# Improbable-AI/walk-these-ways

Hardware: NVIDIA H100
Metric: env_steps_per_s (higher is better)
Workload: dtype tf32

## Files before the change

include/go1_b200.h:

```cpp
#ifndef GO1_B200_H
#define GO1_B200_H
#include <stdint.h>
#ifdef __cplusplus
extern "C" {
#endif

#define GO1_NUM_DOF 12
#define GO1_NUM_COMMANDS 15
#define GO1_MAX_OBS 128
#define GO1_MAX_PRIV_OBS 48
#define GO1_EVENT_STRIDE 6
#define GO1_RESET_RAND_STRIDE 48
#define GO1_MAX_LAG_TIMESTEPS 32

enum Go1RewardTerm {
    GO1_REW_TRACKING_LIN_VEL = 0, GO1_REW_TRACKING_ANG_VEL, GO1_REW_LIN_VEL_Z, GO1_REW_ANG_VEL_XY,
    GO1_REW_ORIENTATION, GO1_REW_TORQUES, GO1_REW_DOF_ACC, GO1_REW_ACTION_RATE, GO1_REW_COLLISION,
    GO1_REW_DOF_POS_LIMITS, GO1_REW_JUMP, GO1_REW_TRACKING_CONTACTS_SHAPED_FORCE,
    GO1_REW_TRACKING_CONTACTS_SHAPED_VEL, GO1_REW_DOF_POS, GO1_REW_DOF_VEL, GO1_REW_ACTION_SMOOTHNESS_1,
    GO1_REW_ACTION_SMOOTHNESS_2, GO1_REW_FEET_SLIP, GO1_REW_FEET_CONTACT_VEL, GO1_REW_FEET_CONTACT_FORCES,
    GO1_REW_FEET_CLEARANCE_CMD_LINEAR, GO1_REW_FEET_IMPACT_VEL, GO1_REW_ORIENTATION_CONTROL,
    GO1_REW_RAIBERT_HEURISTIC, GO1_REW_TERMINATION, GO1_NUM_REWARD_TERMS
};

// ... 195 lines not shown
} Go1TailProblem;
int go1_mlp_tail_forward_grouped(const Go1TailProblem* probs, int nprob, int M, int K1, int N2, int N3, void* stream);

int go1_gemm_timing(int on, double* total_ms, double* total_flop, long long* launches);
void go1_kernel_launch_add(long long n);
int go1_transpose(const float* src, int lds, float* dst, int ldd, int rows, int cols, void* stream);
int go1_elu_backward(const float* y, int ldy, const float* dy, int lddy, float* dz, int lddz, int M, int N, void* stream);
int go1_act_backward(const float* y, int ldy, const float* dy, int lddy, float* dz, int lddz, int M, int N, int kind, void* stream);
int go1_mlp_extra_forward(float* y, int ldy, const float* extra, int ldex, const float* w_extra, int ldw, int M, int o, int E, int act,
                          void* stream);
int go1_mlp_extra_backward(const float* dz, int lddz, int dz_transposed, const float* extra, int ldex, const float* w_extra, int ldw,
                           float* g_w_extra, int ldgw, float* dextra, int ldde, int M, int o, int E, int accumulate, void* stream);
int go1_skinny_forward(const float* x, int ldx, const float* W, int ldw, const float* b, float* out, int ldo, int M, int o, int K, void* stream);
int go1_skinny_dgrad(const float* dz, int lddz, const float* W, int ldw, const float* y_prev, int ldy, float* dprev, int lddp,
                     int M, int o, int n, void* stream);
int go1_skinny_dgrad_ex(const float* dz, int lddz, const float* W, int ldw, const float* y_prev, int ldy, float* dprev, int lddp,
                        float* colsum, int M, int o, int n, void* stream);
int go1_skinny_dgrad_act(const float* dz, int lddz, const float* W, int ldw, const float* y_prev, int ldy, float* dprev, int lddp,
                         float* colsum, int M, int o, int n, int kind, void* stream);
int go1_skinny_wgrad_ex(const float* dz, int lddz, const float* x, int ldx, float* gW, int ldg, float* gb, int M, int o, int K, int accumulate, void* stream);
int go1_skinny_wgrad(const float* dz, int lddz, const float* x, int ldx, float* gW, int ldg, int M, int o, int K, int accumulate, void* stream);
typedef struct Go1CopySeg { const float* src; int32_t lds; float* dst; int32_t ldd; int32_t rows, cols; } Go1CopySeg;
int go1_copy_segments(const Go1CopySeg* segs, int n, void* stream);
int go1_colsum(const float* x, int ldx, float* out, int M, int N, int accumulate, void* stream);

int go1_ppo_sample_actions(const float* mean, int ldm, const float* std, const float* eps, uint64_t seed,
                           uint64_t counter, uint64_t* counter_dev, float* actions, float* logp, int n, int num_actions,
                           void* stream);

int go1_ppo_loss(const float* mean, int ldm, const float* std, const float* value, const float* actions,
                 const float* old_logp, const float* old_mean, const float* old_std, const float* advantages,
                 const float* returns, const float* old_values, float* dmean, int lddm, float* dvalue,
                 float* dstd, float* scalars, int n, int num_actions, float clip_param,
                 float value_loss_coef, float entropy_coef, int use_clipped_value_loss, float inv_count,
                 void* stream);

int go1_ppo_mse(const float* pred, int ldp, const float* target, int ldt, float* dpred, int lddp, float* scalars,
                int n, int num_train, int dim, void* stream);

int go1_ppo_grad_sqnorm(const float* grad, int64_t count, double* grad_sq, void* stream);
int go1_ppo_adam_step(float* param, const float* grad, float* exp_avg, float* exp_avg_sq, int64_t count,
                      const double* grad_sq, float max_grad_norm, float lr, const float* lr_dev, float beta1, float beta2,
                      float eps, int step, void* stream);
int go1_ppo_adaptive_lr(const float* scalars, float* lr_dev, float desired_kl, float lr_min, float lr_max, void* stream);

int go1_store_transition(const float* const* in_f32, const uint8_t* dones, const uint8_t* time_outs, float* const* out_f32, uint8_t* s_dones,
// ... 18 lines not shown
```

walk-these-ways_b200/csrc/gemm_tf32.cu:

```cuda
#include <cuda_runtime.h>
#include <cuda.h>
#include <stdint.h>
#include <stdio.h>
#include <mutex>
#include <unordered_map>
#include <stdlib.h>
#include "../../include/go1_b200.h"
#include "wgmma_tf32.cuh"
#include "activation.cuh"

extern int go1_set_error(const char* m);
void go1_count_launch(int n);

namespace {

constexpr int BM = 128, BK = 32;
constexpr int NCONS = 8, EPI_G = 2;

__device__ __forceinline__ uint32_t smem_u32(const void* p) { return (uint32_t)__cvta_generic_to_shared(p); }

__device__ __forceinline__ void mbar_init(uint64_t* bar, uint32_t count) {
    asm volatile("mbarrier.init.shared::cta.b64 [%0], %1;" ::"r"(smem_u32(bar)), "r"(count));
}
__device__ __forceinline__ void mbar_expect_tx(uint64_t* bar, uint32_t bytes) {
// ... 65 lines not shown


struct GemmArgs {
    float* C; const float* bias;
    int M, N, K, ldc, act, kind, accumulate, kb_per_split;
    const float* ex; const float* wex; const float* aux;
    int ldex, ldwex, nex, ldaux;
    int lead;
    int amn, bmn;
    int ct;
    float* colsum;
    const float* bx; const float* bwx; float* gwx; float* dx;
    int ldbx, ldbwx, ldgwx, lddx, nbx;
    int tma_store, tma_aux;
    float* Cg[4]; int nprob, tiles_per_prob;
};
constexpr int GEMM_MAXP = 4;
struct GemmMaps { CUtensorMap a[GEMM_MAXP], b[GEMM_MAXP], half; };

struct EpiStage {
    uint8_t* out;
    const CUtensorMap* mapC;
    const uint8_t* aux;
};
__device__ __forceinline__ void tma_store_2d(const CUtensorMap* map, const void* src, int c0, int c1) {
    asm volatile("cp.async.bulk.tensor.2d.global.shared::cta.bulk_group [%0, {%2, %3}], [%1];"
                 ::"l"(map), "r"(smem_u32(src)), "r"(c0), "r"(c1) : "memory");
}

template <typename D>
__device__ __forceinline__ void epilogue_dact(const D dact, const GemmArgs& g, float (&v)[32], const int row, const int col0, const int ncols, const int lane,
                                              const float4 (&ypre)[8], const bool have_pre, const EpiStage& es) {
    const float* arow = g.aux + (size_t)row * g.ldaux + col0;
    if (es.aux) {
        const uint8_t* srow = es.aux + lane * 128;
#pragma unroll
        for (int j = 0; j < 8; j++) {
            const float4 y = *reinterpret_cast<const float4*>(srow + ((j ^ (lane & 7)) << 4));
            v[4 * j] *= dact(y.x); v[4 * j + 1] *= dact(y.y); v[4 * j + 2] *= dact(y.z); v[4 * j + 3] *= dact(y.w);
        }
    } else if (have_pre) {
#pragma unroll
        for (int j = 0; j < 8; j++) {
            const float4 y = ypre[j];
            v[4 * j] *= dact(y.x); v[4 * j + 1] *= dact(y.y); v[4 * j + 2] *= dact(y.z); v[4 * j + 3] *= dact(y.w);
        }
// ... 82 lines not shown
    }
    if (g.bias) {
        const float bl = cj < g.N ? __ldg(g.bias + cj) : 0.f;
#pragma unroll
        for (int j = 0; j < 32; j++) v[j] += __shfl_sync(0xffffffffu, bl, j);
    }
    const int kind = ANYKIND ? g.kind : (int)GO1_ACT_ELU;
    if (row_ok) {
    if (g.act == 1) {
        const int nlead = g.lead <= 0 ? 32 : max(0, min(32, g.lead - col0));
        GO1_ACT_SWITCH(kind, KD,
            _Pragma("unroll")
            for (int j = 0; j < 32; j++) if (j < nlead) v[j] = act_fast<KD>(v[j]);)
    } else if (g.act == 2) {
        if (ANYKIND) epilogue_dact(act_deriv_coefficients(kind), g, v, row, col0, ncols, lane, ypre, have_pre, es);
        else epilogue_dact([](float y) { return act_deriv<GO1_ACT_ELU>(y); }, g, v, row, col0, ncols, lane, ypre, have_pre, es);
    }
    }
    if (g.colsum) {
        float sred[32];
#pragma unroll
        for (int j = 0; j < 32; j++) sred[j] = (row_ok && j < ncols) ? v[j] : 0.f;
        const float s = transpose_reduce32(sred, lane);
        if (lane < ncols) atomicAdd(g.colsum + col0 + lane, s);
    }
    if (g.nbx > 0) {
        const int cjx = col0 + lane;
#pragma unroll
        for (int t = 0; t < 4; t++) {
            if (t < g.nbx) {
                if (g.gwx) {
                const float e = row_ok ? __ldg(g.bx + (size_t)row * g.ldbx + t) : 0.f;
                float sred[32];
#pragma unroll
                for (int j = 0; j < 32; j++) sred[j] = (row_ok && j < ncols) ? v[j] * e : 0.f;
                const float s = transpose_reduce32(sred, lane);
                if (lane < ncols) atomicAdd(g.gwx + (size_t)cjx * g.ldgwx + t, s);
                }
                if (g.dx) {
                    const float wl = lane < ncols ? __ldg(g.bwx + (size_t)cjx * g.ldbwx + t) : 0.f;
                    float acc = 0.f;
#pragma unroll
                    for (int j = 0; j < 32; j++) acc = fmaf(v[j], __shfl_sync(0xffffffffu, wl, j), acc);
                    if (row_ok) atomicAdd(g.dx + (size_t)row * g.lddx + t, acc);
                }
            }
        }
// ... 17 lines not shown
            else tma_store_2d(es.mapC, es.out, col0, row);
            asm volatile("cp.async.bulk.commit_group;" ::: "memory");
        }
        return;
    }
    if (!row_ok) return;
    if (vec) {
#pragma unroll
        for (int j = 0; j < 8; j++) reinterpret_cast<float4*>(crow)[j] = make_float4(v[4 * j], v[4 * j + 1], v[4 * j + 2], v[4 * j + 3]);
    } else {
#pragma unroll
        for (int j = 0; j < 32; j++) if (j < ncols) crow[j] = v[j];
    }
}

__device__ __forceinline__ bool epilogue_prefetch(const GemmArgs& g, const int row, const int col0, const bool split, float4 (&ypre)[8]) {
    if (g.act != 2 || split || col0 + 32 > g.N || (g.ldaux & 3) != 0 || ((((uintptr_t)g.aux) & 15) != 0) || (col0 & 3) != 0) return false;
    const float4* arow = reinterpret_cast<const float4*>(g.aux + (size_t)(row < g.M ? row : 0) * g.ldaux + col0);
#pragma unroll
    for (int j = 0; j < 8; j++) ypre[j] = __ldg(arow + j);
    return true;
}

constexpr int X_BYTES = 65536;
template <int BN, bool ANYKIND, int CL>
__global__ void __launch_bounds__(32 * NCONS + 128, 1) gemm_tf32_wgmma(const __grid_constant__ GemmMaps gm,
                                                                      const __grid_constant__ CUtensorMap mapC, const __grid_constant__ CUtensorMap mapY, const GemmArgs g,
                                                                      const int tiles_m, const int tiles_n, const int total_tiles, const int stages) {
    static_assert(CL == 1 || (CL == 2 && BN == BM), "CTA pairs share 128-row operand boxes");
    constexpr int G = EPI_G;
    constexpr int A_BYTES = BM * BK * 4, STAGE_BYTES = (BM + BN) * BK * 4;
    constexpr int MAX_STAGES = 8;
    extern __shared__ __align__(1024) uint8_t smem_raw[];
    uint8_t* base = (uint8_t*)(((uintptr_t)smem_raw + 1023) & ~(uintptr_t)1023);
    uint8_t* ring = base;
    uint8_t* xreg = base + (size_t)stages * STAGE_BYTES;
    uint8_t* stage_aux = xreg + X_BYTES;
    uint64_t* full = (uint64_t*)(stage_aux + (g.tma_aux ? NCONS * 4096 : 0));
    uint64_t* empty = full + MAX_STAGES;
    uint64_t* aux_bar = empty + MAX_STAGES;

    const int warp = threadIdx.x >> 5, lane = threadIdx.x & 31;
    const int num_kb_total = (g.K + BK - 1) / BK;

    if (threadIdx.x == 0) {
        for (int p = 0; p < g.nprob; p++) {
            asm volatile("prefetch.tensormap [%0];" ::"l"(&gm.a[p]) : "memory");
            asm volatile("prefetch.tensormap [%0];" ::"l"(&gm.b[p]) : "memory");
        }
        if (g.tma_store) asm volatile("prefetch.tensormap [%0];" ::"l"(&mapC) : "memory");
        if (g.tma_aux) asm volatile("prefetch.tensormap [%0];" ::"l"(&mapY) : "memory");
        if (CL > 1) asm volatile("prefetch.tensormap [%0];" ::"l"(&gm.half) : "memory");
        for (int s = 0; s < stages; s++) { mbar_init(&full[s], 1); mbar_init(&empty[s], CL * NCONS); }
        for (int w = 0; w < NCONS; w++) mbar_init(&aux_bar[w], 1);
        asm volatile("fence.mbarrier_init.release.cluster;" ::: "memory");
    }
    if (CL > 1) cluster_sync();
    else __syncthreads();

    const int npt = total_tiles / CL;
    auto first = [] { return (int)blockIdx.x / CL; };
    auto step = [] { return (int)gridDim.x / CL; };
    auto rank = [] { return CL > 1 ? cluster_ctarank() : 0u; };
    auto pair_n = [&] { return (tiles_n & 1) == 0; };
    auto cta_tile = [&](int pt) -> int {
        if (CL == 1) return pt;
        if (pair_n()) return 2 * pt + (int)rank();
        const int tn = pt % tiles_n, r = pt / tiles_n, hm = tiles_m / 2;
        return ((r / hm) * tiles_m + 2 * (r % hm) + (int)rank()) * tiles_n + tn;
    };
    auto tile_coords = [&](int t, int& m0, int& n0, int& kb0, int& nkb) {
        if (CL == 1 && g.nprob > 1) t %= g.tiles_per_prob;
        const int tn = t % tiles_n; t /= tiles_n;
        const int tm = t % tiles_m; const int z = t / tiles_m;
        m0 = tm * BM; n0 = tn * BN; kb0 = z * g.kb_per_split; nkb = min(g.kb_per_split, num_kb_total - kb0);
    };

    if (warp == NCONS) {
        if (elect_one()) {
// ... 55 lines not shown
    };
    auto release = [&](int s) {
        if (lane == 0) {
            mbar_arrive(&empty[s]);
            if (CL > 1) mbar_arrive_cluster(&empty[s], rank() ^ 1);
        }
    };
    auto request_aux = [&]() {
        if (next_chunk() && lane == 0) {
            int m0, n0, kb0, nkb; tile_coords(cta_tile(pt), m0, n0, kb0, nkb);
            mbar_expect_tx(my_bar, 4096);
            tma_load_2d(&mapY, my_bar, my_aux, n0 + 32 * pc, m0 + 32 * q);
        }
    };
    if (st_aux) request_aux();
    uint32_t aux_phase = 0;
    int s = 0, ph = 0;
    float acc[BN / 2];
    for (int tp = first(); tp < npt; tp += step()) {
        const int t = cta_tile(tp);
        int m0, n0, kb0, nkb; tile_coords(t, m0, n0, kb0, nkb);
        if (st_out && lane == 0) asm volatile("cp.async.bulk.wait_group.read 0;" ::: "memory");
        cons_sync();
        int prev = -1;
        for (int i = 0; i < nkb; i++) {
            mbar_wait(&full[s], ph);
            const uint8_t* a = ring + (size_t)s * STAGE_BYTES;
            const uint8_t* b = a + A_BYTES;
            if (tr) {
                if (g.amn) { uint8_t* ta = xreg + (i & 1) * A_BYTES; transpose_tile<BM>((const float*)a, ta, ctid); a = ta; }
                if (g.bmn) { uint8_t* tb = xreg + 2 * A_BYTES + (i & 1) * A_BYTES; transpose_tile<BN>((const float*)b, tb, ctid); b = tb; }
                if (prev >= 0) {
                    wg::wait<0>();
                    release(prev);
                }
                fence_async_smem();
                cons_sync();
            }
            wg::fence();
            wg::mma_kblock<BN>(acc, a + (size_t)wgi * 64 * 128, b, i > 0);
            wg::commit();
            if (!tr && prev >= 0) {
                wg::wait<1>();
                release(prev);
            }
            prev = s;
// ... 1 lines not shown
        }
        wg::wait<0>();
        release(prev);
        if (tr) cons_sync();

        const int row = m0 + 32 * q + lane;
        float* const Cbase = CL == 1 && g.nprob > 1 ? g.Cg[t / g.tiles_per_prob] : g.C;
        float4 ypre[8];
        const bool have_pre = CL == 1 && !st_aux && (grp < BN / 32) && epilogue_prefetch(g, row, n0 + 32 * grp, split, ypre);
        store_fragment<BN / 8>(acc, xwg, 0, w, lane, [](float2 v, int, int) { return v; });
        wg_sync(wgi);
#pragma unroll 1
        for (int c = grp; c < BN / 32; c += G) {
            if (n0 + 32 * c >= g.N) break;
            uint8_t* blk = xwg + (size_t)c * (64 * 128) + (w & 1) * 4096;
            uint32_t r[32];
            const uint8_t* srow = blk + lane * 128;
#pragma unroll
            for (int j = 0; j < 8; j++) {
                const uint4 x = *reinterpret_cast<const uint4*>(srow + ((j ^ (lane & 7)) << 4));
                r[4 * j] = x.x; r[4 * j + 1] = x.y; r[4 * j + 2] = x.z; r[4 * j + 3] = x.w;
            }
            EpiStage es;
            es.out = st_out ? blk : nullptr; es.mapC = &mapC; es.aux = st_aux ? my_aux : nullptr;
            if (st_aux) { mbar_wait(my_bar, aux_phase); aux_phase ^= 1; }
            epilogue_chunk<ANYKIND>(g, Cbase, r, row, n0 + 32 * c, split, lane, ypre, have_pre && c == grp, es);
            if (st_aux) { __syncwarp(); request_aux(); }
        }
    }
    if (st_out && lane == 0) asm volatile("cp.async.bulk.wait_group 0;" ::: "memory");
    if (CL > 1) cluster_sync();
}

typedef CUresult (*EncodeTiledFn)(CUtensorMap*, CUtensorMapDataType, cuuint32_t, void*, const cuuint64_t*, const cuuint64_t*, const cuuint32_t*,
                                  const cuuint32_t*, CUtensorMapInterleave, CUtensorMapSwizzle, CUtensorMapL2promotion, CUtensorMapFloatOOBfill);
EncodeTiledFn g_encode = nullptr;
std::once_flag g_once;

int sm_count() {
    static int sms = 0;
    if (!sms) { int dev = 0; cudaGetDevice(&dev); cudaDeviceGetAttribute(&sms, cudaDevAttrMultiProcessorCount, dev); if (sms <= 0) sms = 132; }
    return sms;
}

int make_map_uncached(CUtensorMap* map, const float* ptr, int rows, int cols, int ld, int box_rows, int box_cols, CUtensorMapSwizzle swz);
struct MapKey { const float* ptr; int rows, cols, ld, box_rows, box_cols, swz; bool operator==(const MapKey& o) const { return ptr == o.ptr && rows == o.rows && cols == o.cols && ld == o.ld && box_rows == o.box_rows && box_cols == o.box_cols && swz == o.swz; } };
struct MapKeyHash { size_t operator()(const MapKey& k) const { size_t h = (size_t)k.ptr; h = h * 1000003u ^ (size_t)k.rows; h = h * 1000003u ^ (size_t)k.cols; h = h * 1000003u ^ (size_t)k.ld; h = h * 1000003u ^ (size_t)(k.box_rows * 8 + k.swz); h = h * 1000003u ^ (size_t)k.box_cols; return h; } };
std::unordered_map<MapKey, CUtensorMap, MapKeyHash> g_map_cache;
std::mutex g_map_mutex;
int make_map(CUtensorMap* map, const float* ptr, int rows, int cols, int ld, int box_rows, int box_cols = BK, CUtensorMapSwizzle swz = CU_TENSOR_MAP_SWIZZLE_128B) {
    const MapKey key{ptr, rows, cols, ld, box_rows, box_cols, (int)swz};
// ... 40 lines not shown
    }
    return best;
}

__global__ void zero_strided(float* C, int ldc, int M, int N) {
    const size_t i = (size_t)blockIdx.x * blockDim.x + threadIdx.x;
    if (i >= (size_t)M * N) return;
    C[(i / N) * ldc + (i % N)] = 0.f;
}
__global__ void bias_act_strided(float* C, int ldc, const float* bias, int M, int N, int act, int kind) {
    const size_t i = (size_t)blockIdx.x * blockDim.x + threadIdx.x;
    if (i >= (size_t)M * N) return;
    float* c = C + (i / N) * ldc + (i % N);
    float v = *c;
    if (bias) v += bias[i % N];
    if (act == 1) { GO1_ACT_SWITCH(kind, KD, v = act_exact<KD>(v);) }
    *c = v;
}

template <int BN, bool ANYKIND, int CL>
int launch_gemm(const GemmMaps& gm, const CUtensorMap& mc, const CUtensorMap& my, GemmArgs& g, int splits, cudaStream_t st) {
    constexpr int STAGE_BYTES = (BM + BN) * BK * 4;
    const size_t staging = X_BYTES + (g.tma_aux ? (size_t)NCONS * 4096 : 0);
    const size_t fixed = staging + (2 * 8 + NCONS) * 8 + 16 + 1024;
    const size_t budget = 227 * 1024;
    int stages = (int)((budget - fixed) / STAGE_BYTES);
    if (stages > 8) stages = 8;
    if (stages < 2) return go1_set_error("go1_gemm impl=1: no room for the operand ring");
    const size_t smem = (size_t)stages * STAGE_BYTES + fixed;
    auto kernel = gemm_tf32_wgmma<BN, ANYKIND, CL>;
    const int tiles_m = (g.M + BM - 1) / BM, tiles_n = (g.N + BN - 1) / BN;
    g.tiles_per_prob = tiles_m * tiles_n * splits;
    const int total = g.tiles_per_prob * (g.nprob > 1 ? g.nprob : 1);
    cudaLaunchConfig_t cfg = {};
    cudaLaunchAttribute attr[1];
    attr[0].id = cudaLaunchAttributeClusterDimension;
    attr[0].val.clusterDim.x = CL; attr[0].val.clusterDim.y = 1; attr[0].val.clusterDim.z = 1;
    cfg.blockDim = dim3(32 * NCONS + 128); cfg.dynamicSmemBytes = smem; cfg.stream = st;
    cfg.attrs = attr; cfg.numAttrs = 1;
    static bool configured = false;
    static int slots = 0;
    if (!configured) {
        cudaError_t e = cudaFuncSetAttribute(kernel, cudaFuncAttributeMaxDynamicSharedMemorySize, (int)budget);
        if (e != cudaSuccess) return go1_set_error(cudaGetErrorString(e));
        slots = sm_count();
        if (CL > 1) {
            cfg.gridDim = dim3(CL * sm_count());
// ... 351 lines not shown
    else if (BN == 64) e = any ? launch_gemm<64, true, 1>(gm, mc, my, g, splits, st) : launch_gemm<64, false, 1>(gm, mc, my, g, splits, st);
    else e = any ? launch_gemm<32, true, 1>(gm, mc, my, g, splits, st) : launch_gemm<32, false, 1>(gm, mc, my, g, splits, st);
    if (e) return e;
    if (splits > 1 && (bias || act))
        for (int p = 0; p < nprob; p++) { const size_t tot = (size_t)M * N; bias_act_strided<<<(unsigned)((tot + 255) / 256), 256, 0, st>>>(Cs[p], ldc, bias, M, N, act, ep->act_kind); go1_count_launch(1); }
    if (timed) cudaEventRecord(timing_event(), st);
    cudaError_t ce = cudaGetLastError();
    if (ce != cudaSuccess) return go1_set_error(cudaGetErrorString(ce));
    return 0;
}

extern "C" int go1_gemm_tf32(int transA, int transB, int M, int N, int K, const float* A, int lda, const float* B, int ldb,
                             float* Cm, int ldc, const Go1GemmEpilogue* ep, cudaStream_t st) {
    return gemm_tf32_impl(transA, transB, M, N, K, 1, &A, lda, &B, ldb, &Cm, ldc, ep, st);
}
extern "C" int go1_gemm_grouped(int transA, int transB, int M, int N, int K, int nprob, const float* const* A, int lda, const float* const* B, int ldb,
                                float* const* C, int ldc, int accumulate, void* stream) {
    if (!A || !B || !C || nprob < 1 || nprob > GEMM_MAXP || M <= 0 || N <= 0 || K <= 0) return go1_set_error("go1_gemm_grouped: 1..4 problems");
    Go1GemmEpilogue ep = {};
    ep.accumulate = accumulate;
    return gemm_tf32_impl(transA, transB, M, N, K, nprob, A, lda, B, ldb, C, ldc, &ep, (cudaStream_t)stream);
}

__global__ void transpose_kernel(const float* __restrict__ src, int lds, float* __restrict__ dst, int ldd, int rows, int cols) {
    __shared__ float t[32][33];
    const int c0 = blockIdx.x * 32, r0 = blockIdx.y * 32;
    for (int i = threadIdx.y; i < 32; i += 8) {
        const int r = r0 + i, c = c0 + threadIdx.x;
        t[i][threadIdx.x] = (r < rows && c < cols) ? src[(size_t)r * lds + c] : 0.f;
    }
    __syncthreads();
    for (int i = threadIdx.y; i < 32; i += 8) {
        const int c = c0 + i, r = r0 + threadIdx.x;
        if (c < cols && r < rows) dst[(size_t)c * ldd + r] = t[threadIdx.x][i];
    }
}
extern "C" int go1_transpose(const float* src, int lds, float* dst, int ldd, int rows, int cols, void* stream) {
    if (!src || !dst || rows <= 0 || cols <= 0 || lds < cols || ldd < rows) return go1_set_error("go1_transpose: bad arguments");
    dim3 grid((cols + 31) / 32, (rows + 31) / 32);
    transpose_kernel<<<grid, dim3(32, 8), 0, (cudaStream_t)stream>>>(src, lds, dst, ldd, rows, cols);
    go1_count_launch(1);
    cudaError_t ce = cudaGetLastError();
    if (ce != cudaSuccess) return go1_set_error(cudaGetErrorString(ce));
    return 0;
}


extern "C" int go1_mlp_tail_forward_grouped(const Go1TailProblem* probs, int nprob, int M, int K1, int N2, int N3, void* stream) {
    cudaStream_t st = (cudaStream_t)stream;
    if (!probs || nprob < 1 || nprob > TAIL_MAXP || M <= 0) return go1_set_error("go1_mlp_tail_forward: 1 or 2 problems of the same shape");
    const bool shape_a = (K1 == 512 && N2 == 256 && N3 == 128), shape_b = (K1 == 256 && N2 == 128 && N3 == 0);
    if (!shape_a && !shape_b) return go1_set_error("go1_mlp_tail_forward: supported tails are 512-256-128-head and 256-128-head");
    TailMaps maps;
    TailArgs g;
    g.nprob = nprob; g.M = M; g.tiles_per_prob = (M + TAIL_BM - 1) / TAIL_BM; g.tiles = g.tiles_per_prob * nprob;
    g.kind = probs[0].act_kind;
    if (!go1_act_kind_ok(g.kind)) return go1_set_error("go1_mlp_tail_forward: unknown activation kind (Go1Activation)");
    int rows = 0;
    for (int p = 0; p < nprob; p++) {
        const Go1TailProblem& q = probs[p];
        if (q.act_kind != g.kind) return go1_set_error("go1_mlp_tail_forward: the problems of one launch share their activation kind");
        if (!q.x || !q.W2 || !q.y2 || !q.Wh || !q.out || q.nh < 1 || q.nh > TAIL_HPW || q.ldout < q.nh) return go1_set_error("go1_mlp_tail_forward: bad arguments (head width 1..12)");
        if (N3 > 0 && (!q.W3 || !q.y3)) return go1_set_error("go1_mlp_tail_forward: the three-layer tail needs W3 / y3");
        if ((q.ldx & 3) || (q.ldy2 & 3) || (N3 > 0 && (q.ldy3 & 3)) ||
            ((((uintptr_t)q.x | (uintptr_t)q.W2 | (uintptr_t)q.y2 | (uintptr_t)(N3 > 0 ? (const void*)q.W3 : (const void*)q.W2) |
               (uintptr_t)(N3 > 0 ? (const void*)q.y3 : (const void*)q.y2)) & 15) != 0))
            return go1_set_error("go1_mlp_tail_forward: operands must be 16-byte aligned with row strides that are multiples of 4 floats");
        if (int e = make_map(&maps.x[p], q.x, M, K1, q.ldx, TAIL_BM)) return e;
        if (int e = make_map(&maps.w2[p], q.W2, N2, K1, K1, N2)) return e;
// ... 34 lines not shown
```

walk-these-ways_b200/go1_b200/capi.py:

```python
import ctypes as C
import os

_PKG = os.path.dirname(os.path.dirname(os.path.abspath(__file__)))
LIB_PATH = os.path.join(_PKG, "lib", "libgo1b200.so")

NUM_DOF = 12
NUM_COMMANDS = 15
MAX_OBS = 128
MAX_PRIV_OBS = 48
EVENT_STRIDE = 6
XR_STRIDE = 8

REWARD_TERMS = [
    "tracking_lin_vel", "tracking_ang_vel", "lin_vel_z", "ang_vel_xy", "orientation", "torques", "dof_acc",
    "action_rate", "collision", "dof_pos_limits", "jump", "tracking_contacts_shaped_force",
    "tracking_contacts_shaped_vel", "dof_pos", "dof_vel", "action_smoothness_1", "action_smoothness_2",
    "feet_slip", "feet_contact_vel", "feet_contact_forces", "feet_clearance_cmd_linear", "feet_impact_vel",
    "orientation_control", "raibert_heuristic", "termination",
]
NUM_REWARD_TERMS = len(REWARD_TERMS)
NUM_EPISODE_SUMS = NUM_REWARD_TERMS + 1
NUM_COMMAND_SUMS = NUM_REWARD_TERMS + 5
COMMAND_SUM_EXTRAS = ["lin_vel_raw", "ang_vel_raw", "lin_vel_residual", "ang_vel_residual", "ep_timesteps"]

# ... 95 lines not shown
                ("ld_w_extra", _i), ("num_extra", _i), ("dact_y", C.c_void_p), ("ld_dact_y", _i), ("lead_cols", _i), ("colsum", C.c_void_p),
                ("bwd_extra", C.c_void_p), ("bwd_w_extra", C.c_void_p), ("g_w_extra", C.c_void_p), ("d_extra", C.c_void_p),
                ("ld_bwd_extra", _i), ("ld_bwd_w_extra", _i), ("ld_g_w_extra", _i), ("ld_d_extra", _i), ("num_bwd_extra", _i), ("act_kind", _i),
                ("store_transposed", _i)]


class Go1TailProblem(C.Structure):
    _fields_ = [("x", C.c_void_p), ("ldx", _i), ("W2", C.c_void_p), ("b2", C.c_void_p), ("y2", C.c_void_p), ("ldy2", _i),
                ("W3", C.c_void_p), ("b3", C.c_void_p), ("y3", C.c_void_p), ("ldy3", _i), ("Wh", C.c_void_p), ("bh", C.c_void_p), ("nh", _i),
                ("out", C.c_void_p), ("ldout", _i), ("act_kind", _i)]


class Go1CopySeg(C.Structure):
    _fields_ = [("src", C.c_void_p), ("lds", _i), ("dst", C.c_void_p), ("ldd", _i), ("rows", _i), ("cols", _i)]


def copy_segments(pairs):
    n = len(pairs)
    arr = (Go1CopySeg * n)()
    for sg, (dst, src) in zip(arr, pairs):
        assert dst.shape == src.shape and dst.dim() == 2 and dst.stride(1) == 1 and src.stride(1) == 1
        sg.src, sg.lds, sg.dst, sg.ldd, sg.rows, sg.cols = src.data_ptr(), src.stride(0), dst.data_ptr(), dst.stride(0), dst.shape[0], dst.shape[1]
    check(lib().go1_copy_segments(arr, n, stream_ptr()), "go1_copy_segments")


class Go1Error(RuntimeError):
    pass


_lib = None


def lib():
    global _lib
    if _lib is not None:
        return _lib
    if not os.path.exists(LIB_PATH):
        raise Go1Error(f"{LIB_PATH} not found: build it with `python -c 'import __graft_entry__ as g; g.build()'` "
                       f"(nvcc, sm_90a). There is no CPU fallback.")
    L = C.CDLL(LIB_PATH)
    L.go1_last_error.restype = C.c_char_p
    vp, ip, i64 = C.c_void_p, C.c_int, C.c_int64
    sig = {
        "go1_version": ([], ip), "go1_device_count": ([], ip), "go1_sizeof_config": ([], ip), "go1_sizeof_buffers": ([], ip),
        "go1_kernel_launch_count": ([], C.c_longlong), "go1_kernel_launch_add": ([C.c_longlong], None),
        "go1_gemm_timing": ([ip, C.POINTER(C.c_double), C.POINTER(C.c_double), C.POINTER(C.c_longlong)], ip),
# ... 8 lines not shown
        "go1_sizeof_curriculum": ([ip], ip), "go1_curriculum_set_grouped": ([ip], None),
        "go1_curriculum_resample": ([vp, C.POINTER(Go1CurriculumConfig), C.POINTER(Go1CurriculumBuffers), ip, vp], ip),
        "go1_curriculum_pack": ([vp, C.POINTER(Go1CurriculumConfig), C.POINTER(Go1CurriculumBuffers), vp], ip),
        "go1_sim_reset_idx_dev": ([vp, vp, vp, vp, vp, ip, i64, vp, vp], ip),
        "go1_history_roll": ([vp, vp, vp, ip, ip, ip, vp], ip),
        "go1_history_roll_pitched": ([vp, ip, vp, vp, ip, ip, ip, ip, vp], ip),
        "go1_ppo_gae": ([vp, vp, vp, vp, vp, vp, vp, ip, ip, _f, _f, vp], ip),
        "go1_ppo_normalize_advantages": ([vp, vp, i64, i64, vp], ip),
        "go1_gemm": ([ip, ip, ip, ip, ip, vp, ip, vp, ip, vp, ip, vp, ip, ip, ip, vp], ip),
        "go1_gemm_ex": ([ip, ip, ip, ip, ip, vp, ip, vp, ip, vp, ip, C.POINTER(Go1GemmEpilogue), ip, vp], ip),
        "go1_mlp_tail_forward_grouped": ([C.POINTER(Go1TailProblem), ip, ip, ip, ip, ip, vp], ip),
        "go1_mlp_tail_forward": ([vp, ip, ip, ip, vp, vp, ip, vp, ip, vp, vp, ip, vp, ip, vp, vp, ip, vp, ip, vp], ip),
        "go1_transpose": ([vp, ip, vp, ip, ip, ip, vp], ip),
        "go1_elu_backward": ([vp, ip, vp, ip, vp, ip, ip, ip, vp], ip),
        "go1_act_backward": ([vp, ip, vp, ip, vp, ip, ip, ip, ip, vp], ip),
        "go1_mlp_extra_forward": ([vp, ip, vp, ip, vp, ip, ip, ip, ip, ip, vp], ip),
        "go1_mlp_extra_backward": ([vp, ip, ip, vp, ip, vp, ip, vp, ip, vp, ip, ip, ip, ip, ip, vp], ip),
        "go1_skinny_dgrad": ([vp, ip, vp, ip, vp, ip, vp, ip, ip, ip, ip, vp], ip),
        "go1_skinny_dgrad_ex": ([vp, ip, vp, ip, vp, ip, vp, ip, vp, ip, ip, ip, vp], ip),
        "go1_skinny_dgrad_act": ([vp, ip, vp, ip, vp, ip, vp, ip, vp, ip, ip, ip, ip, vp], ip),
        "go1_skinny_wgrad_ex": ([vp, ip, vp, ip, vp, ip, vp, ip, ip, ip, ip, vp], ip),
        "go1_gemm_grouped": ([ip, ip, ip, ip, ip, ip, C.POINTER(vp), ip, C.POINTER(vp), ip, C.POINTER(vp), ip, ip, vp], ip),
        "go1_copy_segments": ([C.POINTER(Go1CopySeg), ip, vp], ip),
        "go1_skinny_forward": ([vp, ip, vp, ip, vp, vp, ip, ip, ip, ip, vp], ip),
        "go1_skinny_wgrad": ([vp, ip, vp, ip, vp, ip, ip, ip, ip, ip, vp], ip),
        "go1_colsum": ([vp, ip, vp, ip, ip, ip, vp], ip),
        "go1_ppo_sample_actions": ([vp, ip, vp, vp, C.c_uint64, C.c_uint64, vp, vp, vp, ip, ip, vp], ip),
        "go1_ppo_loss": ([vp, ip, vp, vp, vp, vp, vp, vp, vp, vp, vp, vp, ip, vp, vp, vp, ip, ip, _f, _f, _f, ip, _f, vp], ip),
        "go1_ppo_mse": ([vp, ip, vp, ip, vp, ip, vp, ip, ip, ip, vp], ip),
        "go1_ppo_grad_sqnorm": ([vp, i64, vp, vp], ip),
        "go1_ppo_adam_step": ([vp, vp, vp, vp, i64, vp, _f, _f, vp, _f, _f, _f, ip, vp], ip),
        "go1_ppo_adaptive_lr": ([vp, vp, _f, _f, _f, vp], ip),
        "go1_store_transition": ([vp, vp, vp, vp, vp, ip, ip, ip, ip, ip, _f, vp], ip),
        "go1_store_observations": ([vp, vp, vp, vp, ip, ip, ip, vp], ip),
        "go1_rollout_store_observations": ([vp, vp, vp, vp, vp, ip, ip, ip, vp], ip),
        "go1_rollout_store_transition": ([vp, vp, vp, vp, vp, vp, ip, ip, ip, ip, ip, _f, vp], ip),
        "go1_rollout_advance": ([vp, vp, ip, ip, vp, vp, vp], ip),
        "go1_gather_rows": ([vp, vp, vp, i64, ip, ip, vp], ip),
    }
    for name, (args, res) in sig.items():
        fn = getattr(L, name)
        fn.argtypes = args
        fn.restype = res
    if L.go1_sizeof_config() != C.sizeof(Go1SimConfig):
        raise Go1Error(f"Go1SimConfig mirror out of date: C {L.go1_sizeof_config()} vs ctypes {C.sizeof(Go1SimConfig)}")
    if L.go1_sizeof_buffers() != C.sizeof(Go1SimBuffers):
# ... 34 lines not shown
```

walk-these-ways_b200/go1_gym_learn/ppo_cse/actor_critic.py:

```python
import torch
import torch.nn as nn
from params_proto import PrefixProto

from go1_b200 import capi


class AC_Args(PrefixProto, cli=False):
    init_noise_std = 1.0
    actor_hidden_dims = [512, 256, 128]
    critic_hidden_dims = [512, 256, 128]
    activation = 'elu'
    adaptation_module_branch_hidden_dims = [256, 128]
    use_decoder = False
    gemm_impl = 1


def _mlp(in_dim, hidden, out_dim, activation):
    layers, d = [], in_dim
    for h in hidden:
        layers += [nn.Linear(d, h), get_activation(activation)]
        d = h
    layers.append(nn.Linear(d, out_dim))
    return nn.Sequential(*layers)

# ... 193 lines not shown
            elif skinny:
                capi.check(L.go1_skinny_wgrad(capi.ptr(dz), ldz, capi.ptr(inp), ld_in, gW.data_ptr(), i, M, o, K, 1, st), "skinny_wgrad")
            else:
                tc = impl == 1 and M >= 64 and K >= 8 and self._tma_ok(dz, ldz) and self._tma_ok(inp, ld_in)
                if tc and wgrads is not None:
                    wgrads.append((o, K, M, ldz, ld_in, i, dz, inp, gW))
                else:
                    self._gemm(1, 0, o, K, M, dz, ldz, inp, ld_in, gW, i, None, 0, 1 if tc else 0, 1 if tc else 0)
            if li == 0:
                if extra is not None and not extra_done and (want_dextra or dz1T is None):
                    E = i - K0
                    if want_dextra:
                        dextra = self._buf((tag, "dextra"), M, E)
                    gwx = gW.data_ptr() + 4 * K0 if dz1T is None else None
                    capi.check(L.go1_mlp_extra_backward(capi.ptr(dz), ldz, 0 if dz1T is None else 1, capi.ptr(extra), extra.stride(0), W.data_ptr() + 4 * K0, i,
                                                        gwx, i, capi.ptr(dextra) if want_dextra else None, E, M, o, E, 0, st), "extra_backward")
                return dextra
            pwo, pbo, po, pi = self.specs[li - 1]
            gb_prev, yprev = self.grad[pbo:pbo + po], outs[li - 1]
            to_T = li == 1 and dz1T is not None
            dprev = dz1T if to_T else self._buf((tag, "d", li - 1), M, i)
            ldp = dprev.stride(0)
            if impl == 1 and self._tma_ok(dz, ldz) and self._tma_ok(W, i) and M >= 64:
                bx = None
                if li == 1 and extra is not None and 1 <= pi - K0 <= 4:
                    extra_done = True
                    if want_dextra:
                        dextra = self._buf((tag, "dextra"), M, pi - K0).zero_()
                    gwx = None if to_T else self.grad.data_ptr() + 4 * (pwo + K0)
                    if dextra is not None or gwx is not None:
                        bx = (extra, self.flat.data_ptr() + 4 * (pwo + K0), pi, gwx, pi, dextra)
                self._gemm(0, 0, M, i, o, dz, ldz, W, i, dprev, ldp, None, 2, 0, 1, dact_y=yprev, colsum=None if to_T else gb_prev, bwd_extra=bx,
                           store_transposed=1 if to_T else 0)
                bias_done = True
            elif to_T:
                raise capi.Go1Error("transposed first-layer dz: the dgrad that produces it must be a tensor-core product")
            elif o <= 16:
                bias_done = impl == 1 and i % 4 == 0 and self._tma_ok(W, i) and self._tma_ok(dprev, ldp) and self._tma_ok(yprev, yprev.stride(0))
                capi.check(L.go1_skinny_dgrad_act(capi.ptr(dz), ldz, capi.ptr(W), i, capi.ptr(yprev), yprev.stride(0), capi.ptr(dprev), ldp,
                                                  gb_prev.data_ptr() if bias_done else None, M, o, i, self.kind, st), "skinny_dgrad")
            else:
                self._gemm(0, 0, M, i, o, dz, ldz, W, i, dprev, ldp, None, 2, 0, 0, dact_y=yprev)
                bias_done = False
            dz = dprev


class ActorCritic(nn.Module):
    is_recurrent = False
    HEAD = 16
    MAX_PRIVILEGED_OBS = 64

    def __init__(self, num_obs, num_privileged_obs, num_obs_history, num_actions, **kwargs):
        if kwargs:
            print("ActorCritic.__init__ got unexpected arguments, which will be ignored: " + str([key for key in kwargs.keys()]))
        self.decoder = AC_Args.use_decoder
        super().__init__()
# ... 41 lines not shown
        ps = self._ordered_params()
        dev = ps[0].device
        offsets, off = {}, self.HEAD
        for p in ps:
            off = (off + 3) // 4 * 4
            offsets[id(p)] = off
            off += p.numel()
        total = (off + 3) // 4 * 4
        flat = torch.zeros(total, device=dev, dtype=torch.float32)
        for p in ps:
            o, n = offsets[id(p)], p.numel()
            flat[o:o + n].copy_(p.data.reshape(-1))
            p.data = flat[o:o + n].view(p.shape)
        self._flat = flat
        self._packed_version = -1
        self._grad = torch.zeros_like(flat)
        self.n_params = total
        self._nets = {}
        for name, seq in (("adapt", self.adaptation_module), ("actor", self.actor_body), ("critic", self.critic_body)):
            self._nets[name] = _Net(seq, self._flat, self._grad, offsets, self)
        self.n_adapt_params = (self._nets["adapt"].end + 3) // 4 * 4
        self.std_offset = offsets[id(self.std)]

    def ensure_packed(self):
        if self._flat is None or self._packed_version == self.weights_version:
            return
        for net in self._nets.values():
            net.refresh_packed()
        self._packed_version = self.weights_version

    @property
    def flat_params(self):
        self.flatten()
        return self._flat

    @property
    def flat_grads(self):
        self.flatten()
        return self._grad

    def load_state_dict(self, *a, **k):
        self.flatten()
        self.weights_version += 1
        return super().load_state_dict(*a, **k)

    def reset(self, dones=None):
# ... 224 lines not shown
        for name in names:
            xcol = {"adapt": None, "actor": K0 + 1 + E, "critic": K0 + 1}[name]
            wo, bo, o, i = nets[name].specs[0]
            gW = self._grad[wo:wo + o * i].view(o, i)
            pairs.append((gW[:, :K0], gcat[row:row + o, :K0]))
            pairs.append((self._grad[bo:bo + o].view(o, 1), gcat[row:row + o, K0:K0 + 1]))
            if xcol is not None:
                pairs.append((gW[:, K0:K0 + E], gcat[row:row + o, xcol:xcol + E]))
            row += o
        capi.copy_segments(pairs)

    def backward_ppo(self, h, priv, dmean, dvalue, dstd, hT=None):
        M, K0 = h.shape[0], self.num_obs_history
        nets = self._nets
        self._grad[self.HEAD:].zero_()
        if self._first_layers_fusable(h, priv):
            oa, op, oc = nets["adapt"].specs[0][2], nets["actor"].specs[0][2], nets["critic"].specs[0][2]
            E = self.num_privileged_obs
            if hT is None:
                hT = history_kmajor(h, priv, nets["adapt"]._buf(("train", "hT"), K0 + 1 + 2 * E, (M + 31) // 32 * 32))
            L, st = capi.lib(), capi.stream_ptr()
            capi.check(L.go1_transpose(capi.ptr(self._latent), self._latent.stride(0), capi.ptr(hT[K0 + 1 + E:]), hT.stride(0), M, E, st), "transpose")
            dz1 = nets["adapt"]._buf(("train", "dz1catT"), oa + op + oc, hT.stride(0))
            impl = 1
            wgrads = []
            side = self._side_stream(M)
            if side is not None:
                self._fork(side)
                with torch.cuda.stream(side):
                    nets["critic"].backward(h, h.stride(0), K0, priv, self._c_out, dvalue, M, impl, tag="train", dz1T=dz1[oa + op:], wgrads=wgrads)
            dlat = nets["actor"].backward(h, h.stride(0), K0, self._latent, self._p_out, dmean, M, impl, want_dextra=True, tag="train", dz1T=dz1[oa:oa + op],
                                          wgrads=wgrads)
            if side is None:
                nets["critic"].backward(h, h.stride(0), K0, priv, self._c_out, dvalue, M, impl, tag="train", dz1T=dz1[oa + op:], wgrads=wgrads)
            nets["adapt"].backward(h, h.stride(0), K0, None, self._a_out, dlat, M, impl, tag="train", dz1T=dz1[:oa], wgrads=wgrads)
            if side is not None:
                self._join(side)
            self._flush_wgrads(wgrads)
            self._first_layer_wgrad(("adapt", "actor", "critic"), dz1, hT, M, "train")
        else:
            impl = self._impl()
            dlat = nets["actor"].backward(h, h.stride(0), K0, self._latent, self._p_out, dmean, M, impl, want_dextra=True, tag="train")
            nets["critic"].backward(h, h.stride(0), K0, priv, self._c_out, dvalue, M, impl, tag="train")
            nets["adapt"].backward(h, h.stride(0), K0, None, self._a_out, dlat, M, impl, tag="train")
        self._grad[self.std_offset:self.std_offset + self.num_actions].copy_(dstd)

# ... 25 lines not shown
```

Measured before the change: 1.662 million.

## Use pre-transposed weights for dgrad GEMMs and stage bias colsums in shared memory

```diff
diff --git a/include/go1_b200.h b/include/go1_b200.h
--- a/include/go1_b200.h
+++ b/include/go1_b200.h
@@ -241,6 +241,8 @@
 int go1_skinny_wgrad(const float* dz, int lddz, const float* x, int ldx, float* gW, int ldg, int M, int o, int K, int accumulate, void* stream);
 typedef struct Go1CopySeg { const float* src; int32_t lds; float* dst; int32_t ldd; int32_t rows, cols; } Go1CopySeg;
 int go1_copy_segments(const Go1CopySeg* segs, int n, void* stream);
+#define GO1_MAX_TRANSPOSE_SEGS 16
+int go1_transpose_segments(const Go1CopySeg* segs, int n, void* stream);
 int go1_colsum(const float* x, int ldx, float* out, int M, int N, int accumulate, void* stream);
 
 int go1_ppo_sample_actions(const float* mean, int ldm, const float* std, const float* eps, uint64_t seed,
diff --git a/walk-these-ways_b200/csrc/gemm_tf32.cu b/walk-these-ways_b200/csrc/gemm_tf32.cu
--- a/walk-these-ways_b200/csrc/gemm_tf32.cu
+++ b/walk-these-ways_b200/csrc/gemm_tf32.cu
@@ -111,6 +111,7 @@
     uint8_t* out;
     const CUtensorMap* mapC;
     const uint8_t* aux;
+    float* csum;
 };
 __device__ __forceinline__ void tma_store_2d(const CUtensorMap* map, const void* src, int c0, int c1) {
     asm volatile("cp.async.bulk.tensor.2d.global.shared::cta.bulk_group [%0, {%2, %3}], [%1];"
@@ -239,7 +240,7 @@
 #pragma unroll
         for (int j = 0; j < 32; j++) sred[j] = (row_ok && j < ncols) ? v[j] : 0.f;
         const float s = transpose_reduce32(sred, lane);
-        if (lane < ncols) atomicAdd(g.colsum + col0 + lane, s);
+        if (lane < ncols) atomicAdd(es.csum + lane, s);
     }
     if (g.nbx > 0) {
         const int cjx = col0 + lane;
@@ -303,7 +304,15 @@
     return true;
 }
 
-constexpr int X_BYTES = 65536;
+template <int BN>
+__device__ __forceinline__ void colsum_flush(const GemmArgs& g, float* cs, const int n0, const int ctid) {
+    if (ctid < BN) {
+        if (n0 + ctid < g.N) atomicAdd(g.colsum + n0 + ctid, cs[ctid]);
+        cs[ctid] = 0.f;
+    }
+}
+
+constexpr int X_BYTES = 65536, CS_BYTES = 1024;
 template <int BN, bool ANYKIND, int CL>
 __global__ void __launch_bounds__(32 * NCONS + 128, 1) gemm_tf32_wgmma(const __grid_constant__ GemmMaps gm,
                                                                       const __grid_constant__ CUtensorMap mapC, const __grid_constant__ CUtensorMap mapY, const GemmArgs g,
@@ -314,8 +323,9 @@
     constexpr int MAX_STAGES = 8;
     extern __shared__ __align__(1024) uint8_t smem_raw[];
     uint8_t* base = (uint8_t*)(((uintptr_t)smem_raw + 1023) & ~(uintptr_t)1023);
-    uint8_t* ring = base;
-    uint8_t* xreg = base + (size_t)stages * STAGE_BYTES;
+    float* cs = (float*)base;
+    uint8_t* ring = base + CS_BYTES;
+    uint8_t* xreg = ring + (size_t)stages * STAGE_BYTES;
     uint8_t* stage_aux = xreg + X_BYTES;
     uint64_t* full = (uint64_t*)(stage_aux + (g.tma_aux ? NCONS * 4096 : 0));
     uint64_t* empty = full + MAX_STAGES;
@@ -336,6 +346,7 @@
         for (int w = 0; w < NCONS; w++) mbar_init(&aux_bar[w], 1);
         asm volatile("fence.mbarrier_init.release.cluster;" ::: "memory");
     }
+    if (threadIdx.x < BN) cs[threadIdx.x] = 0.f;
     if (CL > 1) cluster_sync();
     else __syncthreads();
 
@@ -437,6 +448,10 @@
         int m0, n0, kb0, nkb; tile_coords(t, m0, n0, kb0, nkb);
         if (st_out && lane == 0) asm volatile("cp.async.bulk.wait_group.read 0;" ::: "memory");
         cons_sync();
+        if (g.colsum && tp != first()) {
+            int pm0, pn0, pkb0, pnkb; tile_coords(cta_tile(tp - step()), pm0, pn0, pkb0, pnkb);
+            if (pn0 != n0) { colsum_flush<BN>(g, cs, pn0, ctid); cons_sync(); }
+        }
         int prev = -1;
         for (int i = 0; i < nkb; i++) {
             mbar_wait(&full[s], ph);
@@ -484,11 +499,16 @@
                 r[4 * j] = x.x; r[4 * j + 1] = x.y; r[4 * j + 2] = x.z; r[4 * j + 3] = x.w;
             }
             EpiStage es;
-            es.out = st_out ? blk : nullptr; es.mapC = &mapC; es.aux = st_aux ? my_aux : nullptr;
+            es.out = st_out ? blk : nullptr; es.mapC = &mapC; es.aux = st_aux ? my_aux : nullptr; es.csum = cs + 32 * c;
             if (st_aux) { mbar_wait(my_bar, aux_phase); aux_phase ^= 1; }
             epilogue_chunk<ANYKIND>(g, Cbase, r, row, n0 + 32 * c, split, lane, ypre, have_pre && c == grp, es);
             if (st_aux) { __syncwarp(); request_aux(); }
         }
+    }
+    if (g.colsum && first() < npt) {
+        int pm0, pn0, pkb0, pnkb; tile_coords(cta_tile(first() + (npt - 1 - first()) / step() * step()), pm0, pn0, pkb0, pnkb);
+        cons_sync();
+        colsum_flush<BN>(g, cs, pn0, ctid);
     }
     if (st_out && lane == 0) asm volatile("cp.async.bulk.wait_group 0;" ::: "memory");
     if (CL > 1) cluster_sync();
@@ -575,7 +595,7 @@
 int launch_gemm(const GemmMaps& gm, const CUtensorMap& mc, const CUtensorMap& my, GemmArgs& g, int splits, cudaStream_t st) {
     constexpr int STAGE_BYTES = (BM + BN) * BK * 4;
     const size_t staging = X_BYTES + (g.tma_aux ? (size_t)NCONS * 4096 : 0);
-    const size_t fixed = staging + (2 * 8 + NCONS) * 8 + 16 + 1024;
+    const size_t fixed = CS_BYTES + staging + (2 * 8 + NCONS) * 8 + 16 + 1024;
     const size_t budget = 227 * 1024;
     int stages = (int)((budget - fixed) / STAGE_BYTES);
     if (stages > 8) stages = 8;
@@ -973,9 +993,9 @@
     return gemm_tf32_impl(transA, transB, M, N, K, nprob, A, lda, B, ldb, C, ldc, &ep, (cudaStream_t)stream);
 }
 
-__global__ void transpose_kernel(const float* __restrict__ src, int lds, float* __restrict__ dst, int ldd, int rows, int cols) {
+__device__ __forceinline__ void transpose_block32(const float* __restrict__ src, int lds, float* __restrict__ dst, int ldd, int rows, int cols,
+                                                  int r0, int c0) {
     __shared__ float t[32][33];
-    const int c0 = blockIdx.x * 32, r0 = blockIdx.y * 32;
     for (int i = threadIdx.y; i < 32; i += 8) {
         const int r = r0 + i, c = c0 + threadIdx.x;
         t[i][threadIdx.x] = (r < rows && c < cols) ? src[(size_t)r * lds + c] : 0.f;
@@ -985,6 +1005,9 @@
         const int c = c0 + i, r = r0 + threadIdx.x;
         if (c < cols && r < rows) dst[(size_t)c * ldd + r] = t[threadIdx.x][i];
     }
+}
+__global__ void transpose_kernel(const float* __restrict__ src, int lds, float* __restrict__ dst, int ldd, int rows, int cols) {
+    transpose_block32(src, lds, dst, ldd, rows, cols, blockIdx.y * 32, blockIdx.x * 32);
 }
 extern "C" int go1_transpose(const float* src, int lds, float* dst, int ldd, int rows, int cols, void* stream) {
     if (!src || !dst || rows <= 0 || cols <= 0 || lds < cols || ldd < rows) return go1_set_error("go1_transpose: bad arguments");
@@ -996,6 +1019,34 @@
     return 0;
 }
 
+constexpr int TSEG_MAX = GO1_MAX_TRANSPOSE_SEGS;
+struct TransposeSegs { Go1CopySeg s[TSEG_MAX]; int tile0[TSEG_MAX + 1]; int n; };
+__global__ void transpose_segments_kernel(const __grid_constant__ TransposeSegs a) {
+    int si = 0;
+    while (si + 1 < a.n && (int)blockIdx.x >= a.tile0[si + 1]) si++;
+    const Go1CopySeg& sg = a.s[si];
+    const int tiles_c = (sg.cols + 31) / 32, tl = (int)blockIdx.x - a.tile0[si];
+    transpose_block32(sg.src, sg.lds, sg.dst, sg.ldd, sg.rows, sg.cols, (tl / tiles_c) * 32, (tl % tiles_c) * 32);
+}
+extern "C" int go1_transpose_segments(const Go1CopySeg* segs, int n, void* stream) {
+    if (!segs || n < 1 || n > TSEG_MAX) return go1_set_error("go1_transpose_segments: 1..GO1_MAX_TRANSPOSE_SEGS segments");
+    TransposeSegs a; a.n = n;
+    long long tiles = 0;
+    for (int i = 0; i < n; i++) {
+        const Go1CopySeg& g = segs[i];
+        if (!g.src || !g.dst || g.rows <= 0 || g.cols <= 0 || g.lds < g.cols || g.ldd < g.rows) return go1_set_error("go1_transpose_segments: bad segment");
+        a.s[i] = g;
+        a.tile0[i] = (int)tiles;
+        tiles += (long long)((g.rows + 31) / 32) * ((g.cols + 31) / 32);
+        if (tiles > (1 << 30)) return go1_set_error("go1_transpose_segments: too many tiles");
+    }
+    a.tile0[n] = (int)tiles;
+    transpose_segments_kernel<<<(unsigned)tiles, dim3(32, 8), 0, (cudaStream_t)stream>>>(a);
+    go1_count_launch(1);
+    cudaError_t ce = cudaGetLastError();
+    if (ce != cudaSuccess) return go1_set_error(cudaGetErrorString(ce));
+    return 0;
+}
 
 extern "C" int go1_mlp_tail_forward_grouped(const Go1TailProblem* probs, int nprob, int M, int K1, int N2, int N3, void* stream) {
     cudaStream_t st = (cudaStream_t)stream;
diff --git a/walk-these-ways_b200/go1_b200/capi.py b/walk-these-ways_b200/go1_b200/capi.py
--- a/walk-these-ways_b200/go1_b200/capi.py
+++ b/walk-these-ways_b200/go1_b200/capi.py
@@ -141,6 +141,18 @@
         assert dst.shape == src.shape and dst.dim() == 2 and dst.stride(1) == 1 and src.stride(1) == 1
         sg.src, sg.lds, sg.dst, sg.ldd, sg.rows, sg.cols = src.data_ptr(), src.stride(0), dst.data_ptr(), dst.stride(0), dst.shape[0], dst.shape[1]
     check(lib().go1_copy_segments(arr, n, stream_ptr()), "go1_copy_segments")
+
+
+MAX_TRANSPOSE_SEGS = 16
+
+
+def transpose_segments(pairs):
+    n = len(pairs)
+    arr = (Go1CopySeg * n)()
+    for sg, (dst, src) in zip(arr, pairs):
+        assert dst.shape == src.shape[::-1] and dst.dim() == 2 and dst.stride(1) == 1 and src.stride(1) == 1
+        sg.src, sg.lds, sg.dst, sg.ldd, sg.rows, sg.cols = src.data_ptr(), src.stride(0), dst.data_ptr(), dst.stride(0), src.shape[0], src.shape[1]
+    check(lib().go1_transpose_segments(arr, n, stream_ptr()), "go1_transpose_segments")
 
 
 class Go1Error(RuntimeError):
@@ -195,6 +207,7 @@
         "go1_skinny_wgrad_ex": ([vp, ip, vp, ip, vp, ip, vp, ip, ip, ip, ip, vp], ip),
         "go1_gemm_grouped": ([ip, ip, ip, ip, ip, ip, C.POINTER(vp), ip, C.POINTER(vp), ip, C.POINTER(vp), ip, ip, vp], ip),
         "go1_copy_segments": ([C.POINTER(Go1CopySeg), ip, vp], ip),
+        "go1_transpose_segments": ([C.POINTER(Go1CopySeg), ip, vp], ip),
         "go1_skinny_forward": ([vp, ip, vp, ip, vp, vp, ip, ip, ip, ip, vp], ip),
         "go1_skinny_wgrad": ([vp, ip, vp, ip, vp, ip, ip, ip, ip, ip, vp], ip),
         "go1_colsum": ([vp, ip, vp, ip, ip, ip, vp], ip),
diff --git a/walk-these-ways_b200/go1_gym_learn/ppo_cse/actor_critic.py b/walk-these-ways_b200/go1_gym_learn/ppo_cse/actor_critic.py
--- a/walk-these-ways_b200/go1_gym_learn/ppo_cse/actor_critic.py
+++ b/walk-these-ways_b200/go1_gym_learn/ppo_cse/actor_critic.py
@@ -239,6 +239,7 @@
             dprev = dz1T if to_T else self._buf((tag, "d", li - 1), M, i)
             ldp = dprev.stride(0)
             if impl == 1 and self._tma_ok(dz, ldz) and self._tma_ok(W, i) and M >= 64:
+                WT = self.owner._dgrad_weights()[self, li]
                 bx = None
                 if li == 1 and extra is not None and 1 <= pi - K0 <= 4:
                     extra_done = True
@@ -247,8 +248,8 @@
                     gwx = None if to_T else self.grad.data_ptr() + 4 * (pwo + K0)
                     if dextra is not None or gwx is not None:
                         bx = (extra, self.flat.data_ptr() + 4 * (pwo + K0), pi, gwx, pi, dextra)
-                self._gemm(0, 0, M, i, o, dz, ldz, W, i, dprev, ldp, None, 2, 0, 1, dact_y=yprev, colsum=None if to_T else gb_prev, bwd_extra=bx,
-                           store_transposed=1 if to_T else 0)
+                self._gemm(0, 1, M, i, o, dz, ldz, WT, WT.stride(0), dprev, ldp, None, 2, 0, 1, dact_y=yprev, colsum=None if to_T else gb_prev,
+                           bwd_extra=bx, store_transposed=1 if to_T else 0)
                 bias_done = True
             elif to_T:
                 raise capi.Go1Error("transposed first-layer dz: the dgrad that produces it must be a tensor-core product")
@@ -336,6 +337,26 @@
         self.n_adapt_params = (self._nets["adapt"].end + 3) // 4 * 4
         self.std_offset = offsets[id(self.std)]
 
+    def _dgrad_weights(self):
+        flat = self._flat
+
+        def build(old):
+            if old is None:
+                old = {}
+                for net in self._nets.values():
+                    for li, (wo, bo, o, i) in enumerate(net.specs):
+                        if li >= 1 and _Net._tma_ok(flat[wo:], i):
+                            old[net, li] = _empty(i, (o + 3) // 4 * 4, device=flat.device)[:, :o]
+            pairs = []
+            for (net, li), wt in old.items():
+                wo, _, o, i = net.specs[li]
+                pairs.append((wt, flat[wo:wo + o * i].view(o, i)))
+            for k in range(0, len(pairs), capi.MAX_TRANSPOSE_SEGS):
+                capi.transpose_segments(pairs[k:k + capi.MAX_TRANSPOSE_SEGS])
+            return old
+
+        return self._nets["adapt"]._cached(("wT", "all"), build)
+
     def ensure_packed(self):
         if self._flat is None or self._packed_version == self.weights_version:
             return
@@ -606,6 +627,7 @@
             L, st = capi.lib(), capi.stream_ptr()
             capi.check(L.go1_transpose(capi.ptr(self._latent), self._latent.stride(0), capi.ptr(hT[K0 + 1 + E:]), hT.stride(0), M, E, st), "transpose")
             dz1 = nets["adapt"]._buf(("train", "dz1catT"), oa + op + oc, hT.stride(0))
+            self._dgrad_weights()
             impl = 1
             wgrads = []
             side = self._side_stream(M)
```

Result: no change. 1.677 million (median of 6 runs) (+0.9%).
